# fabianschenk/REVO

Measured on AMD Instinct MI355X. Metric: tracked frames/sec at 640x480, 4-level pyramid; ATE vs reference, higher is better.
Workload: dtype f32

## Files before the change

### profiles/stream_busy.py

```python
import collections
import sqlite3
import statistics
import sys

db = sqlite3.connect(sys.argv[1])
cols = [r[1] for r in db.execute("pragma table_info(kernels)")]
sid = "stream_id" if "stream_id" in cols else "queue_id"
rows = list(db.execute("select name, start, end, %s from kernels order by start" % sid))
short = lambda n: n.replace("(anonymous namespace)::", "").replace("void ", "").split("(")[0]
trk = [i for i, r in enumerate(rows) if "k_track<false>" in r[0]]
first = int(sys.argv[2]) if len(sys.argv) > 2 else 14
count = int(sys.argv[3]) if len(sys.argv) > 3 else 30
t_idx = trk[first:first + count]
t0, t1 = rows[t_idx[0]][1], rows[t_idx[-1]][1]
nsteps = len(t_idx) - 1
print("%d steps between tracker launches %d and %d: %.1f us per step" % (nsteps, first, first + count - 1, (t1 - t0) / 1e3 / nsteps))
busy = collections.defaultdict(float)
dur = collections.defaultdict(list)
by = collections.defaultdict(list)
for n, s, e, q in rows:
    if t0 <= s < t1:
        busy[q] += (e - s) / 1e3
        dur[short(n)].append((e - s) / 1e3)
        by[q].append((s, e, short(n)))
for q in sorted(busy):
    names = collections.Counter(x[2] for x in by[q]).most_common(2)
    print("stream %-3s busy %6.1f us per step  (%s)" % (q, busy[q] / nsteps, ", ".join(n for n, _ in names)))
print("kernel                         per step   avg us   min     max")
for k, v in sorted(dur.items(), key=lambda kv: -sum(kv[1])):
    print("%-30s %6.2f   %7.1f %7.1f %7.1f" % (k, len(v) / nsteps, statistics.mean(v), min(v), max(v)))
print("idle gap in front of a kernel on its own stream (mean / max us):")
for q in sorted(by):
    gaps = collections.defaultdict(list)
    for a, b in zip(by[q], by[q][1:]):
        gaps[b[2]].append((b[0] - a[1]) / 1e3)
    print("  stream %-3s %s" % (q, {k: (round(statistics.mean(v), 1), round(max(v), 1)) for k, v in gaps.items()}))
```

### revo_amd/csrc/revo_dev.h

```cpp
#pragma once
#include <hip/hip_runtime.h>
#include <stdint.h>
#include "../../include/revo_hip.h"

#define REVO_L REVO_MAX_LEVELS

struct LevelGeom {
  int w, h;
  int npix;
  float fx, fy, cx, cy;
  int patch;
  int hist_w, hist_h;
  int nchunk;
  int chunk_rows;
  int wpr;
  int nms_block_base;
  int has_orig;
  int pix_base;
  int edt_rows;
  int edt_block_base;
  int strip_base;
  int cc_base;
  int band_rows, nbands, band_base;
};

struct PyrGeom {
  int frame0;
  int fstride;
  int n_levels;
  int total_nms_blocks, total_pix, total_edt_blocks, total_strips, total_cc;
  int total_bands, any_banded;
  int hyst_force;
  int hyst_heavy_runs;
  int total_tiles;
  int pts_staged;
  float depth_min, depth_max;
  int canny_low, canny_high;
  int use_edge_hist;
  float n_percentage;
  double fill_thr[REVO_L];
  LevelGeom lv[REVO_L];
};

struct FramePlanes {
  uint8_t* gray[REVO_L];
  float* depth[REVO_L];
  uint2* cs[REVO_L];
  uint8_t* edges[REVO_L];
  uint8_t* edges_orig[REVO_L];
  int* scratch[REVO_L];
  float4* pts[REVO_L];
  float4* pts_trk[REVO_L];
  float* dt[REVO_L];
  float4* table[REVO_L];
  uint8_t* hist[REVO_L];
  int* chunk[REVO_L];
  unsigned* cmask[REVO_L];
  uint8_t* vb[REVO_L];
  int* npts;
  int* hist_nz;
  int* strip_tot;
  uint32_t* ebits[REVO_L];
  int* need_full;
  int* hyst_heavy;
  int* tile_base;
  float* stage[REVO_L];
  unsigned short* epre[REVO_L];
  int* stage_base;
};

struct PairDesc {
  const float4* pts[REVO_L];
  const int* npts;
  const float* dt[REVO_L];
  float R[9];
  float T[3];
};

struct TrackParams {
  int pyr_min_lvl, pyr_max_lvl;
  int lvl_begin, lvl_end;
  int check_init;
  int eval_only;
  int kspec[REVO_L];
  int redundant_n;
  float lambda_success_fac, lambda_fail_fac;
  float lambda_initial[REVO_L], step_size_min[REVO_L], convergence_eps[REVO_L];
  int max_its[REVO_L];
  float edge_distance[REVO_L];
  float huber_edge;
  int use_edge_filter;
  struct { float fx, fy, cx, cy; int w, h; } cam[REVO_L];
  int exact_sums;
};

struct EvalOut {
  float A[36];
  float b[6];
  float error;
  float mean_err;
  float sum_w, sum_u;
  int good, bad;
};

#define REVO_MAX_WIDTH 2048
#define NMS_ROWS 6
#define EDT_ROW_PX 1280
#ifndef REVO_HYST_LDS_MAX
#define REVO_HYST_LDS_MAX 158720
#endif
#ifndef TRACK_THREADS
#define TRACK_THREADS 512
#endif
#ifndef TRACK_MAX_CLUSTER
#define TRACK_MAX_CLUSTER 32
#endif
#define TRACK_KMAX 4
#define TRACK_NVAL 48
#define TRACK_NVAL_X 132
#define TRACK_MAIL_NVAL TRACK_NVAL_X

void launch_gray_depth(const PyrGeom& g, const FramePlanes& p, const uint8_t* d_bgr, const float* d_depth_f32,
                       const uint16_t* d_depth_u16, float u16_alpha, int B, hipStream_t s);
void launch_pyrdown(const PyrGeom& g, const FramePlanes& p, int lvl, int B, hipStream_t s, int parts = 3, bool stage_edges = false);
void launch_edge_prefix(const PyrGeom& g, const FramePlanes& p, int B, hipStream_t s);
void launch_canny_nms(const PyrGeom& g, const FramePlanes& p, int B, hipStream_t s);
void launch_hyst(const PyrGeom& g, const FramePlanes& p, int B, hipStream_t s);
void launch_fill(const PyrGeom& g, const FramePlanes& p, int B, hipStream_t s);
void launch_compact(const PyrGeom& g, const FramePlanes& p, int B, hipStream_t s);
void launch_tile_points(const PyrGeom& g, const FramePlanes& p, int B, hipStream_t s, int which = 3);
void launch_pyrdown_bgr(const uint8_t* src, int w, int h, uint8_t* dst, hipStream_t s);
void launch_colored_pcl(const PyrGeom& g, const FramePlanes& p, int frame, int lvl, int dense, const uint8_t* bgr_lvl,
                        int* chunk, unsigned* cmask, int* total, int cap, float* out8, hipStream_t s);
void launch_keyframe(const PyrGeom& g, const FramePlanes& p, int f0, int fstride, int count, hipStream_t s, int which = 3);
int launch_track(const PairDesc* d_descs, const TrackParams& prm, revo_pair_result* d_out, EvalOut* d_eval,
                 int n_pairs, unsigned long long* d_mail, unsigned* epoch_io, int cluster, unsigned* d_resident, hipStream_t s);
void launch_track_gate(unsigned* d_resident, unsigned want, hipStream_t s);
int launch_track_one(const PairDesc& desc, const TrackParams& prm, revo_pair_result* out, EvalOut* eval_out,
                     unsigned long long* d_mail, unsigned* epoch_io, int cluster, unsigned* seq_ptr, unsigned seq_val,
                     unsigned* d_resident, hipStream_t s);
void launch_solve6(const float* d_Ab , int n, float* d_x , hipStream_t s);
int track_blocks_per_cu();
void launch_grad_table(const PyrGeom& g, const FramePlanes& p, int f0, int fstride, int count, hipStream_t s);
struct VoteArgs { float RT[3][12]; const float4* pts[3]; const int* n[3]; };
void launch_vote(const PyrGeom& g, const FramePlanes& curr, int curr_frame, int lvl, int n_clouds, const VoteArgs& va,
                 int* d_marks , int* d_hist8 , unsigned* d_done ,
                 int* h_out8 , unsigned seq_val, int use_orig_edges,
                 hipStream_t s);
void launch_copy_cloud(float4* dst, const float4* src, int* dst_n, const int* src_n, hipStream_t s);
struct VoteDesc {
  float RT[3][12]; const float4* pts[3]; const int* n[3]; int n_clouds;
  const uint8_t* edges; const float* depth;
  int* marks; int* hist8; unsigned* done;
  int* host_out;
};
struct CloudCopyDesc { float4* dst; const float4* src; int* dst_n; const int* src_n; };
struct CopySeg { const void* src; void* dst; size_t bytes; };
void launch_vote_multi(const PyrGeom& g, int lvl, int n, const VoteDesc* d_descs, unsigned seq_val, hipStream_t s);
void launch_copy_cloud_multi(int n, const CloudCopyDesc* d_descs, hipStream_t s);
void launch_copy_segments(int n, const CopySeg* d_segs, hipStream_t s);

#define INFO_THREADS 256
#define INFO_CHUNK 1024
#define INFO_MAX_GROUPS 32
#define INFO_PART_DOUBLES 64
struct InfoParams {
  float fx, fy, cx, cy;
  int w, h;
  float edge_distance, huber_edge;
  int use_edge_filter, level;
};
static inline int info_groups(int npix) {
  const int g = (npix + 8 * INFO_CHUNK - 1) / (8 * INFO_CHUNK);
  return g < 1 ? 1 : (g > INFO_MAX_GROUPS ? INFO_MAX_GROUPS : g);
}
void launch_pair_info(const PairDesc* d_descs, const void* d_pose, int pose_stride, int flag_word, const InfoParams& prm,
                      int n_pairs, double* d_part, int* d_cnt, unsigned* d_ticket, revo_pair_info* d_out, hipStream_t s);
```

### revo_amd/csrc/revo_pyramid.hip

```cpp
#include "revo_dev.h"
#include <type_traits>

namespace {

#ifdef REVO_BUILD_PRIO
#define BUILD_PRIO() __builtin_amdgcn_s_setprio(REVO_BUILD_PRIO)
#else
#define BUILD_PRIO()
#endif

__device__ __forceinline__ int level_of(const PyrGeom& g, int v, int LevelGeom::*base) {
  int l = 0;
#pragma unroll
  for (int k = 1; k < REVO_L; ++k)
    if (k < g.n_levels && v >= g.lv[k].*base) l = k;
  return l;
}
__device__ __forceinline__ int clampi(int v, int lo, int hi) { return v < lo ? lo : (v > hi ? hi : v); }
__device__ __forceinline__ int reflect101(int i, int n) {
  if (i < 0) i = -i;
  if (i >= n) i = 2 * n - 2 - i;
  return i;
}

// ... 199 lines not shown
    lo[k] = __builtin_amdgcn_perm(as_u32(dy), as_u32(dx), 0x05040100u);
    hi[k] = __builtin_amdgcn_perm(as_u32(dy), as_u32(dx), 0x07060302u);
  }
  const uint32_t rv = valid ? ~0u : 0u;
#define MAG2(x) __builtin_amdgcn_sdot2(as_s2(x), as_s2(x), 0, false)
  m.v0 = MAG2(lo[0]) & (int)(cm_left & rv);
  m.v1 = MAG2(hi[0]) & (int)rv;
  m.v2 = MAG2(lo[1]) & (int)rv;
  m.v3 = MAG2(hi[1]) & (int)rv;
  m.v4 = MAG2(lo[2]) & (int)rv;
  m.v5 = MAG2(hi[2]) & (int)(cm_right & rv);
#undef MAG2
  dxy.v0 = hi[0]; dxy.v1 = lo[1]; dxy.v2 = hi[1]; dxy.v3 = lo[2];
}
__device__ __forceinline__ void nms_row4(const MRow4& A, const MRow4& B, const MRow4& C, const DRow4& d, int low, int high,
                                         uint32_t* cand, uint32_t* strong) {
  uint32_t cb = 0, sb = 0;
  nms_px(0, A.v0, A.v1, A.v2, B.v0, B.v1, B.v2, C.v0, C.v1, C.v2, d.v0, low, high, cb, sb);
  nms_px(1, A.v1, A.v2, A.v3, B.v1, B.v2, B.v3, C.v1, C.v2, C.v3, d.v1, low, high, cb, sb);
  nms_px(2, A.v2, A.v3, A.v4, B.v2, B.v3, B.v4, C.v2, C.v3, C.v4, d.v2, low, high, cb, sb);
  nms_px(3, A.v3, A.v4, A.v5, B.v3, B.v4, B.v5, C.v3, C.v4, C.v5, d.v3, low, high, cb, sb);
  *cand = cb;
  *strong = sb;
}
__global__ void __launch_bounds__(256) k_canny_nms4(PyrGeom g, FramePlanes pl) {
  BUILD_PRIO();
  const int f = g.frame0 + blockIdx.z;
  if (blockIdx.x == 0 && threadIdx.x < REVO_L) {
    pl.need_full[f * REVO_L + threadIdx.x] = 0;
    pl.hist_nz[f * REVO_L + threadIdx.x] = 0;
  }
  const int l = level_of(g, blockIdx.x, &LevelGeom::nms_block_base);
  const LevelGeom& lv = g.lv[l];
  const int w = lv.w, h = lv.h;
  const int rt = 8 * lv.wpr;
  const int t = (blockIdx.x - lv.nms_block_base) * 256 + threadIdx.x;
  const int yb = t / rt, xg = t - yb * rt;
  const int y0 = yb * NMS_R;
  if (y0 >= h) return;
  const int x = xg * 4;
  const bool active = x < w;
  const uint8_t* gray = pl.gray[l] + (size_t)f * lv.npix;
  const bool has_prev = x > 0, has_next = x + 4 < w;
  const int xo = active ? x : 0;
  const int o_prev = (active && has_prev) ? xo - 4 : xo, o_next = (active && has_next) ? xo + 4 : xo;
  const uint32_t cm_left = (active && has_prev) ? ~0u : 0u, cm_right = (active && has_next) ? ~0u : 0u;
  struct Raw { uint32_t prev, m0, next; };
  auto load_raw = [&](int r) -> Raw {
    const int rr = clampi(r, 0, h - 1);
    const uint8_t* row = gray + (size_t)rr * w;
    Raw q;
    q.m0 = *reinterpret_cast<const uint32_t*>(row + xo);
    q.prev = *reinterpret_cast<const uint32_t*>(row + o_prev);
    q.next = *reinterpret_cast<const uint32_t*>(row + o_next);
    return q;
  };
  auto make_hrow = [&](Raw q) -> HRow4 {
    if (!has_prev) q.prev = (q.m0 & 0xffu) * 0x01010101u;
    if (!has_next) q.next = (q.m0 >> 24) * 0x01010101u;
    return hrow4(q.prev, q.m0, q.next);
  };
  HRow4 H0, H1, H2;
  MRow4 M0, M1, M2;
  DRow4 D0, D1, D2;
  {
    const Raw r0 = load_raw(y0 - 2), r1 = load_raw(y0 - 1), r2 = load_raw(y0), r3 = load_raw(y0 + 1);
    H0 = make_hrow(r0); H1 = make_hrow(r1); H2 = make_hrow(r2);
    mag_row4(H0, H1, H2, cm_left, cm_right, active && y0 - 1 >= 0, M0, D0);
    H0 = make_hrow(r3);
  }
  Raw ahead = load_raw(y0 + 2);
  mag_row4(H1, H2, H0, cm_left, cm_right, active, M1, D1);
  uint2* out = pl.cs[l] + ((size_t)f * h + y0) * lv.wpr + (xg >> 3);
  const int sh = 4 * (threadIdx.x & 7);
  auto emit = [&](int i, uint32_t cb, uint32_t sb) {
    uint32_t cw = cb << sh, sw = sb << sh;
    cw |= (uint32_t)__builtin_amdgcn_update_dpp(0, (int)cw, 0xB1, 0xf, 0xf, true);
    sw |= (uint32_t)__builtin_amdgcn_update_dpp(0, (int)sw, 0xB1, 0xf, 0xf, true);
    cw |= (uint32_t)__builtin_amdgcn_update_dpp(0, (int)cw, 0x4E, 0xf, 0xf, true);
    sw |= (uint32_t)__builtin_amdgcn_update_dpp(0, (int)sw, 0x4E, 0xf, 0xf, true);
    cw |= (uint32_t)__builtin_amdgcn_update_dpp(0, (int)cw, 0x141, 0xf, 0xf, true);
    sw |= (uint32_t)__builtin_amdgcn_update_dpp(0, (int)sw, 0x141, 0xf, 0xf, true);
    if ((threadIdx.x & 7) == 0 && y0 + i < h) out[(size_t)i * lv.wpr] = make_uint2(cw, sw);
  };
#define NMS_STEP4(i, Ha, Hb, Hc, Ma, Mb, Mc, Db, Dc)                                  \
  {                                                                                   \
    Hc = make_hrow(ahead);                                                            \
    if ((i) < NMS_R - 1) ahead = load_raw(y0 + (i) + 3);                              \
    mag_row4(Ha, Hb, Hc, cm_left, cm_right, active && y0 + (i) + 1 < h, Mc, Dc);      \
    uint32_t cb, sb;                                                                  \
    nms_row4(Ma, Mb, Mc, Db, g.canny_low, g.canny_high, &cb, &sb);                    \
    emit((i), cb, sb);                                                                \
  }
  NMS_STEP4(0, H2, H0, H1, M0, M1, M2, D1, D2)
  NMS_STEP4(1, H0, H1, H2, M1, M2, M0, D2, D0)
  NMS_STEP4(2, H1, H2, H0, M2, M0, M1, D0, D1)
  NMS_STEP4(3, H2, H0, H1, M0, M1, M2, D1, D2)
  NMS_STEP4(4, H0, H1, H2, M1, M2, M0, D2, D0)
  NMS_STEP4(5, H1, H2, H0, M2, M0, M1, D0, D1)
#undef NMS_STEP4
}

#ifndef HYST_THREADS
#define HYST_THREADS 1024
#endif
__device__ __forceinline__ uint32_t dil3(uint32_t a, uint32_t al, uint32_t ar) {
  return a | __builtin_amdgcn_alignbit(a, al, 31) | __builtin_amdgcn_alignbit(ar, a, 1);
}
__device__ __forceinline__ uint32_t run_fill(uint32_t C, uint32_t S) {
  const uint32_t up = ((C + S) ^ C) & C;
  const uint32_t rC = __builtin_bitreverse32(C), rS = __builtin_bitreverse32(S);
  const uint32_t dn = __builtin_bitreverse32(((rC + rS) ^ rC) & rC);
  return up | dn | S;
}

#ifdef REVO_HYST_PROFILE
#define HP(i) if (threadIdx.x == 0) hp[i] = clock64()
#define HA(i) if (threadIdx.x == 0) { const long long now_ = clock64(); ha[i] += now_ - hlast; hlast = now_; }
#else
#define HP(i)
#define HA(i)
#endif
template <bool C_IN_LDS, bool E_GLOBAL = false>
__device__ __forceinline__ void hyst_level(const PyrGeom& g, const FramePlanes& pl, const int l, const int f, uint32_t* s_mem) {
  static_assert(!(C_IN_LDS && E_GLOBAL), "the candidate bitmap is in LDS only when the edge bitmap is");
#ifdef REVO_HYST_PROFILE
  long long hp[12], ha[8], hlast = 0;
  for (int i = 0; i < 12; ++i) hp[i] = 0;
  for (int i = 0; i < 8; ++i) ha[i] = 0;
  int dbg_sweeps = 0, dbg_bands = 0;
#endif
  HP(0);
  const LevelGeom& lv = g.lv[l];
  const int w = lv.w, h = lv.h, wpr = lv.wpr;
  const int pitch = wpr;
  const int nwords = h * wpr;
  const int e_words = (h + 2) * pitch + 2;
  uint32_t* Cl = s_mem;
  uint32_t* Ebase = C_IN_LDS ? s_mem + (REVO_HYST_LDS_MAX / 4 - e_words)
                  : (E_GLOBAL ? reinterpret_cast<uint32_t*>(pl.scratch[l] + (size_t)f * g.lv[l].npix) : s_mem);
  uint32_t* E = Ebase + 1;
  const uint2* cs = pl.cs[l] + (size_t)f * h * wpr;
  const int tid = threadIdx.x;
  for (int i = tid; i < pitch + 1; i += HYST_THREADS) { Ebase[i] = 0u; Ebase[e_words - 1 - i] = 0u; }
  for (int i = tid; i < nwords; i += HYST_THREADS) {
    const uint2 v = cs[i];
    E[pitch + i] = v.y;
    if (C_IN_LDS) Cl[i] = v.x & ~v.y;
  }
  __syncthreads();
  HP(1);
  bool done = false;
#ifdef REVO_HYST_PROFILE
  int dbg_runs = -1, dbg_t = 0, dbg_a = 0;
#endif
  if (C_IN_LDS) {
    unsigned short* Bs = reinterpret_cast<unsigned short*>(Cl + nwords);
    uint32_t* parent = Cl + nwords + (nwords + 2) / 2;
    const int table_words = (int)(REVO_HYST_LDS_MAX / 4) - (nwords + (nwords + 2) / 2);
    const int cap = min(table_words / 2, table_words - e_words);
    const int cap_keep = (table_words - e_words) / 2;
    __shared__ int s_wsum[HYST_THREADS / 64];
    __shared__ int s_total, s_promoted;
#ifdef REVO_HYST_PROFILE
    __shared__ int s_dbg[4];
    if (tid < 4) s_dbg[tid] = 0;
#endif
    auto weak = [&](int wi) -> uint32_t { return Cl[wi]; };
    auto starts = [](uint32_t wk) -> uint32_t { return wk & ~(wk << 1); };
    const float inv_wpr = 1.0f / (float)wpr;
    const uint32_t FLAG = 0x80000000u, IDM = 0x7fffffffu;
#ifdef REVO_HYST_PROFILE
    hlast = clock64();
#endif
    for (int sweep = 0; sweep < 64 && !done; ++sweep) {
#ifdef REVO_HYST_PROFILE
      ++dbg_sweeps;
#endif
      {
        const int wpt = (nwords + HYST_THREADS - 1) / HYST_THREADS;
        const int w0 = min(nwords, tid * wpt), w1 = min(nwords, w0 + wpt);
        int mine = 0;
        for (int wi = w0; wi < w1; ++wi) mine += __popc(starts(weak(wi)));
        int incl = mine;
#pragma unroll
        for (int o = 1; o < 64; o <<= 1) {
          const int v = __shfl_up(incl, o);
          if ((tid & 63) >= o) incl += v;
        }
        __syncthreads();
        if ((tid & 63) == 63) s_wsum[tid >> 6] = incl;
        if (tid == 0) s_promoted = 0;
        __syncthreads();
        int before = incl - mine;
        for (int k = 0; k < (tid >> 6); ++k) before += s_wsum[k];
        if (tid == HYST_THREADS - 1) { s_total = before + mine; Bs[nwords] = (unsigned short)min(65535, before + mine); }
        for (int wi = w0; wi < w1; ++wi) {
          Bs[wi] = (unsigned short)before;
          before += __popc(starts(weak(wi)));
        }
        __syncthreads();
      }
      const int nruns = s_total;
      HA(0);
#ifdef REVO_HYST_PROFILE
      if (sweep == 0) dbg_runs = nruns;
#endif
      if (nruns >= 65536 || cap < 64) break;
      if (nruns == 0) { done = true; break; }
      int nb = (nruns + cap - 1) / cap, band_rows = h;
      for (;; ++nb) {
        band_rows = (h + nb - 1) / nb;
        bool fits = true;
        for (int r0 = 0; r0 < h; r0 += band_rows)
          fits = fits && ((int)Bs[min(h, r0 + band_rows) * wpr] - (int)Bs[r0 * wpr] <= cap);
        if (fits || band_rows == 1) break;
      }
      if (band_rows == 1 && nb > h) break;
      for (int r0 = 0; r0 < h; r0 += band_rows) {
        const int wa = r0 * wpr, wb = min(h, r0 + band_rows) * wpr;
        const int id0 = Bs[wa], nr = (int)Bs[wb] - id0;
        if (nr == 0) continue;
        uint32_t* rec = parent + nr;
        auto id_of = [&](int wi, int bit) -> int { return (int)Bs[wi] - id0 + __popc(starts(weak(wi)) & ((2u << bit) - 1u)) - 1; };
        auto key_of = [](int x) -> uint32_t { return ((((uint32_t)x * 40503u) >> 1) & 0x7fffu) << 16 | (uint32_t)x; };
        auto find = [&](int x) -> int {
          uint32_t p2 = parent[x] & IDM;
          while ((int)(p2 & 0xffffu) != x) {
            const uint32_t gp = parent[p2 & 0xffffu] & IDM;
            if (gp != p2) atomicMin(&parent[x], gp);
            x = (int)(p2 & 0xffffu); p2 = gp;
          }
          return x;
        };
        auto unite = [&](int a2, int b2) {
          for (;;) {
            a2 = find(a2); b2 = find(b2);
            if (a2 == b2) return;
            uint32_t ka = key_of(a2), kb = key_of(b2);
            if (ka > kb) { const int t2 = a2; a2 = b2; b2 = t2; const uint32_t t3 = ka; ka = kb; kb = t3; }
            const uint32_t old = atomicMin(&parent[b2], ka);
            if (old == kb) return;
            b2 = (int)(old & 0xffffu);
          }
        };
        auto run_at = [&](int i, int* wi_out, uint32_t* run_out) {
          const uint32_t rc = rec[i];
          *wi_out = (int)(rc >> 10);
          *run_out = (0xffffffffu >> (31u - (rc & 31u))) << ((rc >> 5) & 31u);
        };
        for (int wi = wa + tid; wi < wb; wi += HYST_THREADS) {
          int me = (int)Bs[wi] - id0;
          const uint32_t wk = weak(wi);
          for (uint32_t m = starts(wk); m; m &= m - 1, ++me) {
            const int bit = __ffs(m) - 1;
            const uint32_t t2 = ~(wk >> bit);
            const int len = t2 ? __ffs(t2) - 1 : 32 - bit;
            parent[me] = key_of(me);
            rec[me] = ((uint32_t)wi << 10) | ((uint32_t)bit << 5) | (uint32_t)(len - 1);
          }
        }
        __syncthreads();
        HA(1);
#ifdef REVO_HYST_PROFILE
        ++dbg_bands;
#endif
        for (int me = tid; me < nr; me += HYST_THREADS) {
          int wi; uint32_t run;
          run_at(me, &wi, &run);
          int r = (int)(((float)wi + 0.5f) * inv_wpr);
          r += (r + 1) * wpr <= wi ? 1 : (r * wpr > wi ? -1 : 0);
          const int c = wi - r * wpr;
          if ((run & 1u) && c > 0 && (weak(wi - 1) >> 31)) unite(me, id_of(wi - 1, 31));
          if (r == r0) continue;
          for (uint32_t a2 = weak(wi - wpr) & (run | (run << 1) | (run >> 1)); a2;) {
            const int ab = __ffs(a2) - 1;
            a2 &= ~(a2 & ~(a2 + (1u << ab)));
            unite(me, id_of(wi - wpr, ab));
          }
          if ((run & 1u) && c > 0 && (weak(wi - wpr - 1) >> 31)) unite(me, id_of(wi - wpr - 1, 31));
          if ((run >> 31) && c < wpr - 1 && (weak(wi - wpr + 1) & 1u)) unite(me, id_of(wi - wpr + 1, 0));
        }
        __syncthreads();
        HA(2);
        for (int me = tid; me < nr; me += HYST_THREADS) parent[me] = key_of(find(me));
        __syncthreads();
        HA(3);
        if (nr > cap_keep) {
          for (int i = tid; i < pitch + 1; i += HYST_THREADS) { Ebase[i] = 0u; Ebase[e_words - 1 - i] = 0u; }
          for (int i0 = tid; i0 < nwords; i0 += 5 * HYST_THREADS) {
            uint2 v[5];
#pragma unroll
            for (int k = 0; k < 5; ++k) v[k] = cs[min(i0 + k * HYST_THREADS, nwords - 1)];
#pragma unroll
            for (int k = 0; k < 5; ++k) {
              const int i = i0 + k * HYST_THREADS;
              if (i < nwords) E[pitch + i] = v[k].y | (v[k].x & ~Cl[i]);
            }
          }
          __syncthreads();
        }
        HA(6);
        for (int wi = wa + tid; wi < wb; wi += HYST_THREADS) {
          const uint32_t wk = weak(wi);
          if (!wk) continue;
          int r = (int)(((float)wi + 0.5f) * inv_wpr);
          r += (r + 1) * wpr <= wi ? 1 : (r * wpr > wi ? -1 : 0);
          const int c = wi - r * wpr;
          const uint32_t lm = c > 0 ? ~0u : 0u, rm = c < wpr - 1 ? ~0u : 0u;
          const uint32_t* Xc = E + pitch + wi;
          const uint32_t sd = dil3(Xc[-pitch], Xc[-pitch - 1] & lm, Xc[-pitch + 1] & rm) | dil3(Xc[pitch], Xc[pitch - 1] & lm, Xc[pitch + 1] & rm) |
                              __builtin_amdgcn_alignbit(Xc[0], Xc[-1] & lm, 31) | __builtin_amdgcn_alignbit(Xc[1] & rm, Xc[0], 1);
          if (!(wk & sd)) continue;
          const uint32_t touched = run_fill(wk, wk & sd);
          int me = (int)Bs[wi] - id0;
          for (uint32_t m = starts(wk); m; m &= m - 1, ++me)
            if (touched & m & (0u - m)) {
              uint32_t* root = &parent[parent[me] & 0xffffu];
#ifdef REVO_HYST_PROFILE
              atomicAdd(&s_dbg[0], 1);
              if (!(*root & FLAG)) atomicAdd(&s_dbg[1], 1);
#endif
              if (!(*root & FLAG)) atomicOr(root, FLAG);
            }
        }
        __syncthreads();
        HA(4);
#ifdef REVO_HYST_PROFILE
        dbg_t = s_dbg[0]; dbg_a = s_dbg[1];
#endif
        bool any = false;
        for (int wi = wa + tid; wi < wb; wi += HYST_THREADS) {
          const uint32_t wk = weak(wi);
          if (!wk) continue;
          int me = (int)Bs[wi] - id0;
          uint32_t prom = 0;
          for (uint32_t m = starts(wk); m; m &= m - 1, ++me)
            if (parent[parent[me] & 0xffffu] & FLAG) prom |= m & (0u - m);
          if (!prom) continue;
          const uint32_t runs = run_fill(wk, prom);
          Cl[wi] = wk & ~runs;
          E[pitch + wi] |= runs;
          any = any || (r0 > 0 && wi < wa + wpr);
        }
        if (any) s_promoted = 1;
        __syncthreads();
        HA(5);
      }
      if (nb == 1 || !s_promoted) done = true;
    }
    __syncthreads();
  }
  if (!done) {
    __shared__ unsigned short s_list[HYST_THREADS];
    __shared__ unsigned char s_act[2][HYST_THREADS];
    __shared__ int s_n;
  const int max_strips = HYST_THREADS / wpr;
  const int rpt = (h + max_strips - 1) / max_strips;
  const int nstrips = (h + rpt - 1) / rpt;
  const int n_items = nstrips * wpr;
  s_act[0][tid] = 0; s_act[1][tid] = 0;
  if (tid == 0) s_n = 0;
  __syncthreads();
  int n_list = n_items;
#ifndef REVO_HYST_MAXIT
#define REVO_HYST_MAXIT 8192
#endif
  for (int it = 0; it < REVO_HYST_MAXIT; ++it) {
    const int wb = it & 1;
    bool changed = false;
    if (tid < n_list) {
      const int item = it == 0 ? tid : (int)s_list[tid];
      const int strip = item / wpr, c = item - strip * wpr;
      const int r0 = strip * rpt, r1 = min(h, r0 + rpt) - 1;
      uint32_t* Ec = E + pitch + c;
      const uint32_t lm = c > 0 ? ~0u : 0u, rm = c < wpr - 1 ? ~0u : 0u;
      auto Cat = [&](int r) -> uint32_t { return C_IN_LDS ? (Cl[r * wpr + c] | Ec[r * pitch]) : cs[r * wpr + c].x; };
      uint32_t prev_d = dil3(Ec[(r0 - 1) * pitch], Ec[(r0 - 1) * pitch - 1] & lm, Ec[(r0 - 1) * pitch + 1] & rm);
      uint32_t cur = Ec[r0 * pitch], cl = Ec[r0 * pitch - 1] & lm, cr = Ec[r0 * pitch + 1] & rm;
      for (int r = r0; r <= r1; ++r) {
        const uint32_t nx = Ec[(r + 1) * pitch], nl = Ec[(r + 1) * pitch - 1] & lm, nr = Ec[(r + 1) * pitch + 1] & rm;
        const uint32_t Cw = Cat(r);
        const uint32_t hz = __builtin_amdgcn_alignbit(cur, cl, 31) | __builtin_amdgcn_alignbit(cr, cur, 1);
        const uint32_t F = run_fill(Cw, cur | (Cw & (prev_d | dil3(nx, nl, nr) | hz)));
        if (F != cur) { Ec[r * pitch] = F; changed = true; }
        prev_d = dil3(F, cl, cr);
        cur = nx; cl = nl; cr = nr;
      }
      prev_d = dil3(cur, cl, cr);
      cur = Ec[r1 * pitch]; cl = Ec[r1 * pitch - 1] & lm; cr = Ec[r1 * pitch + 1] & rm;
      for (int r = r1; r >= r0; --r) {
        const uint32_t nx = Ec[(r - 1) * pitch], nl = Ec[(r - 1) * pitch - 1] & lm, nr = Ec[(r - 1) * pitch + 1] & rm;
        const uint32_t Cw = Cat(r);
        const uint32_t hz = __builtin_amdgcn_alignbit(cur, cl, 31) | __builtin_amdgcn_alignbit(cr, cur, 1);
        const uint32_t F = run_fill(Cw, cur | (Cw & (prev_d | dil3(nx, nl, nr) | hz)));
        if (F != cur) { Ec[r * pitch] = F; changed = true; }
        prev_d = dil3(F, cl, cr);
        cur = nx; cl = nl; cr = nr;
      }
      if (changed) s_act[wb][item] = 1;
    }
    if (!__syncthreads_or(changed ? 1 : 0)) break;
    bool act = false;
    if (tid < n_items) {
      const int strip = tid / wpr, c = tid - strip * wpr;
      const unsigned char* a = s_act[wb];
#pragma unroll
      for (int ds = -1; ds <= 1; ++ds)
#pragma unroll
        for (int dc = -1; dc <= 1; ++dc) {
          const int ss = strip + ds, cc = c + dc;
          if (ss >= 0 && ss < nstrips && cc >= 0 && cc < wpr) act = act || a[ss * wpr + cc] != 0;
        }
    }
    const unsigned long long m = __ballot(act);
    int base = 0;
    if ((tid & 63) == 0 && m) base = atomicAdd(&s_n, __popcll(m));
    base = __shfl(base, 0);
    if (act) s_list[base + __popcll(m & ((1ull << (tid & 63)) - 1ull))] = (unsigned short)tid;
    s_act[wb ^ 1][tid] = 0;
    __syncthreads();
    n_list = s_n;
    __syncthreads();
    if (tid == 0) s_n = 0;
  }
  __syncthreads();
  }
  __syncthreads();
  HP(5);
  uint8_t* edges = pl.edges[l] + (size_t)f * lv.npix;
  uint8_t* orig = lv.has_orig ? pl.edges_orig[l] + (size_t)f * lv.npix : nullptr;
  const bool rows16 = (w & 15) == 0;
  const float inv_w = 1.0f / (float)w;
  for (int i = tid; i < lv.npix / 16; i += HYST_THREADS) {
    const int p = i * 16;
    int y = (int)(((float)p + 0.5f) * inv_w);
    y += (y + 1) * w <= p ? 1 : (y * w > p ? -1 : 0);
    const int x = p - y * w;
    uint32_t o[4];
    if (rows16) {
      const uint32_t bits = (E[(y + 1) * pitch + (x >> 5)] >> (x & 31)) & 0xffffu;
#pragma unroll
      for (int q = 0; q < 4; ++q) o[q] = ((((bits >> (4 * q)) & 0xfu) * 0x00204081u) & 0x01010101u) * 0xffu;
    } else {
#pragma unroll
      for (int q = 0; q < 4; ++q) {
        int xx = x + 4 * q, yy = y;
        while (xx >= w) { xx -= w; yy += 1; }
        const uint32_t bits = (E[(yy + 1) * pitch + (xx >> 5)] >> (xx & 31)) & 0xfu;
        o[q] = ((bits * 0x00204081u) & 0x01010101u) * 0xffu;
      }
    }
    const uint4 v = make_uint4(o[0], o[1], o[2], o[3]);
    *reinterpret_cast<uint4*>(edges + p) = v;
    if (orig) *reinterpret_cast<uint4*>(orig + p) = v;
  }
  {
    uint2* csw = pl.cs[l] + (size_t)f * h * wpr;
    for (int i = tid; i < nwords; i += HYST_THREADS) csw[i].y = E[pitch + i];
  }
  HP(6);
  if (lv.patch > 0) {
    const int ntiles = lv.hist_w * lv.hist_h;
    int nz = 0;
    const float inv_hw = 1.0f / (float)lv.hist_w;
    for (int t0 = 0; t0 < ntiles; t0 += HYST_THREADS) {
      const int t = t0 + tid;
      if (t < ntiles) {
        int ty = (int)(((float)t + 0.5f) * inv_hw);
        ty += (ty + 1) * lv.hist_w <= t ? 1 : (ty * lv.hist_w > t ? -1 : 0);
        const int tx = t - ty * lv.hist_w;
        const int xa = tx * lv.patch, xb = xa + lv.patch;
        const int wa = xa >> 5, wb = (xb - 1) >> 5;
        const uint32_t ma = ~0u << (xa & 31), mb = (xb & 31) ? ~0u >> (32 - (xb & 31)) : ~0u;
        const uint32_t m0 = wa == wb ? ma & mb : ma, m1 = wb > wa + 1 ? ~0u : (wb > wa ? mb : 0u), m2 = wb > wa + 1 ? mb : 0u;
        const int o1 = wb > wa ? 1 : 0, o2 = wb > wa + 1 ? 2 : 0;
        const uint32_t* row = E + (ty * lv.patch + 1) * pitch + wa;
        int cnt = 0;
        for (int y = 0; y < lv.patch; ++y, row += pitch) cnt += __popc(row[0] & m0) + __popc(row[o1] & m1) + __popc(row[o2] & m2);
        const uint8_t v = (uint8_t)(cnt & 255);
        pl.hist[l][(size_t)f * ntiles + t] = v;
        nz += v != 0;
      }
    }
    __shared__ int s_nz;
    if (tid == 0) s_nz = 0;
    __syncthreads();
    if (nz) atomicAdd(&s_nz, nz);
    __syncthreads();
    if (tid == 0) pl.hist_nz[f * REVO_L + l] = s_nz;
  }
#ifdef REVO_HYST_PROFILE
  HP(7);
  if (threadIdx.x == 0 && l == 0 && f < 64)
    printf("hyst f=%d: load %lld uf_total %lld [scan %lld record %lld link %lld compress %lld flag %lld resolve %lld] runs %d sweeps %d bands %d uf %d rebuild %lld out %lld hist %lld touched %d atomics %d\n", f,
           hp[1] - hp[0], hp[5] - hp[1], ha[0], ha[1], ha[2], ha[3], ha[4], ha[5], dbg_runs, dbg_sweeps, dbg_bands, (int)done, ha[6], hp[6] - hp[5], hp[7] - hp[6], dbg_t, dbg_a);
#endif
}
template <bool C_IN_LDS, bool E_GLOBAL = false>
__global__ void __launch_bounds__(HYST_THREADS) k_hyst(PyrGeom g, FramePlanes pl, int only_flagged, int n_frames) {
  BUILD_PRIO();
  extern __shared__ uint32_t s_mem[];
  const int n_items = g.n_levels * n_frames;
  if (only_flagged) {
    __shared__ int s_any;
    if (threadIdx.x == 0) s_any = 0;
    __syncthreads();
    for (int item = threadIdx.x; item < n_items; item += HYST_THREADS)
      if (pl.need_full[(g.frame0 + item % n_frames) * REVO_L + item / n_frames]) s_any = 1;
    __syncthreads();
    if (!s_any) return;
  }
  for (int item = blockIdx.x; item < n_items; item += gridDim.x) {
    const int l = item / n_frames;
    const int f = g.frame0 + item % n_frames;
    if (only_flagged && !pl.need_full[f * REVO_L + l]) continue;
    hyst_level<C_IN_LDS, E_GLOBAL>(g, pl, l, f, s_mem);
    __syncthreads();
  }
}

#ifndef HB_THREADS
#define HB_THREADS 1024
#endif
#ifndef HB_LDS_WORDS
#define HB_LDS_WORDS 16384
#endif
struct BandRef { int l, R0, R1; };
__device__ __forceinline__ BandRef band_ref(const PyrGeom& g, int bi) {
  int l = 0;
#pragma unroll
  for (int k = 1; k < REVO_L; ++k)
    if (k < g.n_levels && bi >= g.lv[k].band_base) l = k;
  const LevelGeom& lv = g.lv[l];
  const int b = bi - lv.band_base;
  BandRef r;
  r.l = l; r.R0 = b * lv.band_rows; r.R1 = min(lv.h, r.R0 + lv.band_rows);
  return r;
}
__device__ __forceinline__ int band_capb(const LevelGeom& lv) {
  const int hb = lv.band_rows, nwb = hb * lv.wpr;
  const int table_words = HB_LDS_WORDS - (nwb + (nwb + 2) / 2);
  const int e_words = (hb + 2) * lv.wpr + 2;
  int cap = min(table_words / 2, table_words - e_words);
  cap = min(cap, 65535);
  const int h_last = lv.h - (lv.nbands - 1) * lv.band_rows;
  cap = min(cap, ((h_last * lv.w - 4 - 2 * lv.wpr) / 8) * 5);
  return max(cap, 0) & ~31;
}
struct BandRec { int* hdr; int* bs_first; int* bs_last; uint32_t* flags; unsigned short* root; uint32_t* rec; };
__device__ __forceinline__ BandRec band_rec(const FramePlanes& pl, const LevelGeom& lv, int l, int f, int R0, int capb) {
  int* base = pl.scratch[l] + (size_t)f * lv.npix + (size_t)R0 * lv.w;
  BandRec r;
  r.hdr = base; r.bs_first = base + 4; r.bs_last = base + 4 + lv.wpr;
  r.flags = reinterpret_cast<uint32_t*>(base + 4 + 2 * lv.wpr);
  r.root = reinterpret_cast<unsigned short*>(base + 4 + 2 * lv.wpr + capb / 32);
  r.rec = reinterpret_cast<uint32_t*>(base + 4 + 2 * lv.wpr + capb / 32 + capb / 2);
  return r;
}

__device__ __forceinline__ void hyst_band(const PyrGeom& g, const FramePlanes& pl, const BandRef br, const int f, uint32_t* s_mem) {
  __shared__ int s_wsum[HB_THREADS / 64];
  __shared__ int s_total;
  const int l = br.l;
  const LevelGeom& lv = g.lv[l];
  const int h = lv.h, wpr = lv.wpr, pitch = wpr;
  const int hb = br.R1 - br.R0, nwb = hb * wpr, e_words = (hb + 2) * pitch + 2;
  const int tid = threadIdx.x;
  uint32_t* Cl = s_mem;
  uint32_t* Ebase = s_mem + (HB_LDS_WORDS - e_words);
  uint32_t* E = Ebase + 1;
  const uint2* cs = pl.cs[l] + ((size_t)f * h + br.R0) * wpr;
  const int capb = band_capb(lv);
  const BandRec rec_out = band_rec(pl, lv, l, f, br.R0, capb);
  auto load_e = [&](bool with_cl) {
    if (tid == 0) { Ebase[0] = 0u; Ebase[e_words - 1] = 0u; }
    for (int c = tid; c < wpr; c += HB_THREADS) {
      E[c] = br.R0 > 0 ? cs[c - wpr].y : 0u;
      E[(hb + 1) * pitch + c] = br.R1 < h ? cs[nwb + c].y : 0u;
    }
    for (int i0 = tid; i0 < nwb; i0 += 4 * HB_THREADS) {
      uint2 v[4];
#pragma unroll
      for (int k = 0; k < 4; ++k) v[k] = cs[min(i0 + k * HB_THREADS, nwb - 1)];
#pragma unroll
      for (int k = 0; k < 4; ++k) {
        const int i = i0 + k * HB_THREADS;
        if (i < nwb) {
          if (with_cl) { E[pitch + i] = v[k].y; Cl[i] = v[k].x & ~v[k].y; }
          else E[pitch + i] = v[k].y | (v[k].x & ~Cl[i]);
        }
      }
    }
  };
  load_e(true);
  __syncthreads();
  unsigned short* Bs = reinterpret_cast<unsigned short*>(Cl + nwb);
  uint32_t* parent = Cl + nwb + (nwb + 2) / 2;
  const int table_words = HB_LDS_WORDS - (nwb + (nwb + 2) / 2);
  const int cap_keep = (table_words - e_words) / 2;
  auto starts = [](uint32_t wk) -> uint32_t { return wk & ~(wk << 1); };
  const float inv_wpr = 1.0f / (float)wpr;
  const uint32_t FLAG = 0x80000000u, IDM = 0x7fffffffu;
  {
    const int wpt = (nwb + HB_THREADS - 1) / HB_THREADS;
    const int w0 = min(nwb, tid * wpt), w1 = min(nwb, w0 + wpt);
    int mine = 0;
    for (int wi = w0; wi < w1; ++wi) mine += __popc(starts(Cl[wi]));
    int incl = mine;
#pragma unroll
    for (int o = 1; o < 64; o <<= 1) {
      const int v = __shfl_up(incl, o);
      if ((tid & 63) >= o) incl += v;
    }
    if ((tid & 63) == 63) s_wsum[tid >> 6] = incl;
    __syncthreads();
    int before = incl - mine;
    for (int k = 0; k < (tid >> 6); ++k) before += s_wsum[k];
    if (tid == HB_THREADS - 1) { s_total = before + mine; Bs[nwb] = (unsigned short)min(65535, before + mine); }
    for (int wi = w0; wi < w1; ++wi) {
      Bs[wi] = (unsigned short)before;
      before += __popc(starts(Cl[wi]));
    }
    __syncthreads();
  }
  const int nr = s_total;
  if (nr > capb) {
    if (tid == 0) { pl.need_full[f * REVO_L + l] = 1; rec_out.hdr[0] = 0; rec_out.hdr[1] = 0; rec_out.hdr[2] = 0; }
    return;
  }
  uint32_t* rec = parent + nr;
  if (nr > 0) {
    auto id_of = [&](int wi, int bit) -> int { return (int)Bs[wi] + __popc(starts(Cl[wi]) & ((2u << bit) - 1u)) - 1; };
    auto key_of = [](int x) -> uint32_t { return ((((uint32_t)x * 40503u) >> 1) & 0x7fffu) << 16 | (uint32_t)x; };
    auto find = [&](int x) -> int {
      uint32_t p2 = parent[x] & IDM;
      while ((int)(p2 & 0xffffu) != x) {
        const uint32_t gp = parent[p2 & 0xffffu] & IDM;
        if (gp != p2) atomicMin(&parent[x], gp);
        x = (int)(p2 & 0xffffu); p2 = gp;
      }
      return x;
    };
    auto unite = [&](int a2, int b2) {
      for (;;) {
        a2 = find(a2); b2 = find(b2);
        if (a2 == b2) return;
        uint32_t ka = key_of(a2), kb = key_of(b2);
        if (ka > kb) { const int t2 = a2; a2 = b2; b2 = t2; const uint32_t t3 = ka; ka = kb; kb = t3; }
// ... 1298 lines not shown
```

Baseline: 114,500.

## Replace atomic union-find linking in hysteresis with forest build plus pointer jumping

For large bands, the hysteresis connected-component step no longer unites every run with all of its neighbours through atomic union-find. Each run first points at a single neighbour, which builds a forest, and the forest is flattened by synchronous pointer-jumping rounds. Only junction runs, those with more than one neighbour, are collected into an LDS list and united afterwards, followed by another round of jumps. The goal is fewer atomics and less serial find chasing. In exchange the change adds block-wide synchronisation per jump round, and falls back to the iterative path when the jumping does not converge.

```diff
diff --git a/profiles/hyst_link_premise.py b/profiles/hyst_link_premise.py
--- /dev/null
+++ b/profiles/hyst_link_premise.py
@@ -0,0 +1,37 @@
+import os
+import pathlib
+import sys
+import tempfile
+
+import numpy as np
+
+ROOT = os.path.dirname(os.path.dirname(os.path.abspath(__file__)))
+sys.path[:0] = [ROOT, os.path.join(ROOT, "tests")]
+import hyst_link_cases as hc
+from oracle import ro
+from revo_amd import synth
+from revo_amd.settings import ImgPyramidSettings
+
+
+def main():
+    tmp = pathlib.Path(tempfile.mkdtemp())
+    exe = hc.build_host(tmp)
+    s = ImgPyramidSettings.scaled(640, 480, 4, hist_patch=(20, 10, 5, 0, 0, 0))
+    cases, names = [], []
+    for seed in range(int(sys.argv[1]) if len(sys.argv) > 1 else 32):
+        p = synth.make_pair(seed, s)
+        for k in ("ref", "curr"):
+            gray = ro.bgr2gray(p[k][0])
+            cand, strong = hc.nms(gray)
+            if seed < 2:
+                assert np.array_equal(hc.flood(cand, strong), ro.canny(gray) > 0), "the suppression differs from the oracle's"
+            cases.append((hc.words(cand & ~strong), hc.words(strong), 0, 64, 2048))
+            names.append("%d %s" % (seed, k))
+    print("frame      runs junctions share depth votes(forest, roots) serial  link == flood fill")
+    for name, (got, want, st) in zip(names, hc.run_host(exe, tmp, cases)):
+        print("%-8s %6d %9d %5.3f %5d %6d %6d %6d  %s" % (name, st["runs"], st["junctions"], st["junctions"] / max(1, st["runs"]), st["depth"],
+                                                      st["rounds1"], st["rounds2"], st["serial"], np.array_equal(got, want)))
+
+
+if __name__ == "__main__":
+    main()
diff --git a/profiles/stream_busy.py b/profiles/stream_busy.py
--- a/profiles/stream_busy.py
+++ b/profiles/stream_busy.py
@@ -8,7 +8,7 @@
 sid = "stream_id" if "stream_id" in cols else "queue_id"
 rows = list(db.execute("select name, start, end, %s from kernels order by start" % sid))
 short = lambda n: n.replace("(anonymous namespace)::", "").replace("void ", "").split("(")[0]
-trk = [i for i, r in enumerate(rows) if "k_track<false>" in r[0]]
+trk = [i for i, r in enumerate(rows) if "k_track<" in r[0]]
 first = int(sys.argv[2]) if len(sys.argv) > 2 else 14
 count = int(sys.argv[3]) if len(sys.argv) > 3 else 30
 t_idx = trk[first:first + count]
diff --git a/revo_amd/csrc/revo_dev.h b/revo_amd/csrc/revo_dev.h
--- a/revo_amd/csrc/revo_dev.h
+++ b/revo_amd/csrc/revo_dev.h
@@ -1,7 +1,107 @@
 #pragma once
+#include <stdint.h>
+#ifndef REVO_HYST_LINK_HOST
 #include <hip/hip_runtime.h>
-#include <stdint.h>
 #include "../../include/revo_hip.h"
+#endif
+
+#ifdef REVO_HYST_LINK_HOST
+#define HYST_FN static inline
+static inline int hyst_popc(uint32_t v) { return __builtin_popcount(v); }
+static inline int hyst_ffs(uint32_t v) { return __builtin_ffs((int)v); }
+static inline uint32_t hyst_atomic_min(uint32_t* p, uint32_t v) { const uint32_t o = *p; if (v < o) *p = v; return o; }
+#else
+#define HYST_FN __device__ __forceinline__
+__device__ __forceinline__ int hyst_popc(uint32_t v) { return __popc(v); }
+__device__ __forceinline__ int hyst_ffs(uint32_t v) { return __ffs(v); }
+__device__ __forceinline__ uint32_t hyst_atomic_min(uint32_t* p, uint32_t v) { return atomicMin(p, v); }
+#endif
+#define HYST_JUNCTION 0x80000000u
+#define HYST_JUMP_ROUNDS 20
+#define HYST_JUMPS_PER_VOTE 8
+#define HYST_SERIAL_RUNS 3
+
+HYST_FN uint32_t hyst_starts(uint32_t wk) { return wk & ~(wk << 1); }
+HYST_FN uint32_t hyst_key(int x) { return ((((uint32_t)x * 40503u) >> 1) & 0x7fffu) << 16 | (uint32_t)x; }
+HYST_FN int hyst_row(int wi, int wpr, float inv_wpr) {
+  int r = (int)(((float)wi + 0.5f) * inv_wpr);
+  r += (r + 1) * wpr <= wi ? 1 : (r * wpr > wi ? -1 : 0);
+  return r;
+}
+HYST_FN void hyst_run_at(uint32_t rc, int* wi, uint32_t* run) {
+  *wi = (int)((rc & ~HYST_JUNCTION) >> 10);
+  *run = (0xffffffffu >> (31u - (rc & 31u))) << ((rc >> 5) & 31u);
+}
+struct HystWords { uint32_t wl, wu, wul, wur; int bl, bu, bul, bur; };
+HYST_FN HystWords hyst_words(const uint32_t* Cl, const unsigned short* Bs, int wi, int wpr, float inv_wpr, int r0, int id0) {
+  const int r = hyst_row(wi, wpr, inv_wpr), c = wi - r * wpr;
+  const bool up = r > r0, left = c > 0, right = c < wpr - 1;
+  const int il = left ? wi - 1 : wi, iu = up ? wi - wpr : wi, iul = up && left ? wi - wpr - 1 : wi, iur = up && right ? wi - wpr + 1 : wi;
+  HystWords q;
+  q.wl = Cl[il]; q.wu = Cl[iu]; q.wul = Cl[iul]; q.wur = Cl[iur];
+  q.bl = (int)Bs[il] - id0; q.bu = (int)Bs[iu] - id0; q.bul = (int)Bs[iul] - id0; q.bur = (int)Bs[iur] - id0;
+  if (!left) q.wl = 0u;
+  if (!up) q.wu = 0u;
+  if (!(up && left)) q.wul = 0u;
+  if (!(up && right)) q.wur = 0u;
+  return q;
+}
+struct HystNb { uint32_t above; int p, d, r; };
+HYST_FN HystNb hyst_neighbours(uint32_t run, const HystWords& q) {
+  HystNb n;
+  n.p = (run & 1u) && (q.wl >> 31) ? q.bl + hyst_popc(hyst_starts(q.wl)) - 1 : -1;
+  uint32_t a = q.wu & (run | (run << 1) | (run >> 1));
+  if (n.p >= 0 && (a & 1u)) a &= a + 1u;
+  n.above = a;
+  n.d = (run & 1u) && n.p < 0 && !(q.wu & 1u) && (q.wul >> 31) ? q.bul + hyst_popc(hyst_starts(q.wul)) - 1 : -1;
+  n.r = (run >> 31) && !(q.wu >> 31) && (q.wur & 1u) ? q.bur : -1;
+  return n;
+}
+HYST_FN int hyst_id_above(const HystWords& q, int bit) { return q.bu + hyst_popc(hyst_starts(q.wu) & ((2u << bit) - 1u)) - 1; }
+HYST_FN uint32_t hyst_first_parent(int me, uint32_t run, const HystWords& q, bool* junction) {
+  const HystNb n = hyst_neighbours(run, q);
+  const int count = (n.p >= 0) + hyst_popc(hyst_starts(n.above)) + (n.d >= 0) + (n.r >= 0);
+  *junction = count > 1;
+  const int first = n.p >= 0 ? n.p : (n.above ? hyst_id_above(q, hyst_ffs(n.above) - 1) : (n.d >= 0 ? n.d : (n.r >= 0 ? n.r : me)));
+  return hyst_key(first);
+}
+HYST_FN bool hyst_jump(uint32_t* parent, int me, uint32_t p, uint32_t gp) {
+  if (gp == p) return false;
+  parent[me] = gp;
+  return true;
+}
+HYST_FN int hyst_find(uint32_t* parent, int x) {
+  uint32_t p2 = parent[x];
+  while ((int)(p2 & 0xffffu) != x) {
+    const uint32_t gp = parent[p2 & 0xffffu];
+    if (gp != p2) hyst_atomic_min(&parent[x], gp);
+    x = (int)(p2 & 0xffffu); p2 = gp;
+  }
+  return x;
+}
+HYST_FN void hyst_unite(uint32_t* parent, int a2, int b2) {
+  for (;;) {
+    a2 = hyst_find(parent, a2); b2 = hyst_find(parent, b2);
+    if (a2 == b2) return;
+    uint32_t ka = hyst_key(a2), kb = hyst_key(b2);
+    if (ka > kb) { const int t2 = a2; a2 = b2; b2 = t2; const uint32_t t3 = ka; ka = kb; kb = t3; }
+    const uint32_t old = hyst_atomic_min(&parent[b2], ka);
+    if (old == kb) return;
+    b2 = (int)(old & 0xffffu);
+  }
+}
+HYST_FN void hyst_unite_all(uint32_t* parent, int me, uint32_t run, const HystWords& q) {
+  const HystNb n = hyst_neighbours(run, q);
+  if (n.p >= 0) hyst_unite(parent, me, n.p);
+  for (uint32_t a2 = n.above; a2;) {
+    const int ab = hyst_ffs(a2) - 1;
+    a2 &= ~(a2 & ~(a2 + (1u << ab)));
+    hyst_unite(parent, me, hyst_id_above(q, ab));
+  }
+  if (n.d >= 0) hyst_unite(parent, me, n.d);
+  if (n.r >= 0) hyst_unite(parent, me, n.r);
+}
+#ifndef REVO_HYST_LINK_HOST
 
 #define REVO_L REVO_MAX_LEVELS
 
@@ -176,3 +276,4 @@
 }
 void launch_pair_info(const PairDesc* d_descs, const void* d_pose, int pose_stride, int flag_word, const InfoParams& prm,
                       int n_pairs, double* d_part, int* d_cnt, unsigned* d_ticket, revo_pair_info* d_out, hipStream_t s);
+#endif
diff --git a/revo_amd/csrc/revo_pyramid.hip b/revo_amd/csrc/revo_pyramid.hip
--- a/revo_amd/csrc/revo_pyramid.hip
+++ b/revo_amd/csrc/revo_pyramid.hip
@@ -375,8 +375,10 @@
   HP(1);
   bool done = false;
 #ifdef REVO_HYST_PROFILE
-  int dbg_runs = -1, dbg_t = 0, dbg_a = 0;
+  int dbg_runs = -1, dbg_t = 0, dbg_a = 0, dbg_nj = 0;
 #endif
+  __shared__ unsigned short s_list[2 * HYST_THREADS];
+  unsigned char (*s_act)[HYST_THREADS] = reinterpret_cast<unsigned char (*)[HYST_THREADS]>(s_list + HYST_THREADS);
   if (C_IN_LDS) {
     unsigned short* Bs = reinterpret_cast<unsigned short*>(Cl + nwords);
     uint32_t* parent = Cl + nwords + (nwords + 2) / 2;
@@ -384,7 +386,8 @@
     const int cap = min(table_words / 2, table_words - e_words);
     const int cap_keep = (table_words - e_words) / 2;
     __shared__ int s_wsum[HYST_THREADS / 64];
-    __shared__ int s_total, s_promoted;
+    __shared__ int s_total, s_promoted, s_nj;
+    bool bailed = false;
 #ifdef REVO_HYST_PROFILE
     __shared__ int s_dbg[4];
     if (tid < 4) s_dbg[tid] = 0;
@@ -392,7 +395,7 @@
     auto weak = [&](int wi) -> uint32_t { return Cl[wi]; };
     auto starts = [](uint32_t wk) -> uint32_t { return wk & ~(wk << 1); };
     const float inv_wpr = 1.0f / (float)wpr;
-    const uint32_t FLAG = 0x80000000u, IDM = 0x7fffffffu;
+    const uint32_t FLAG = 0x80000000u;
 #ifdef REVO_HYST_PROFILE
     hlast = clock64();
 #endif
@@ -445,33 +448,7 @@
         const int id0 = Bs[wa], nr = (int)Bs[wb] - id0;
         if (nr == 0) continue;
         uint32_t* rec = parent + nr;
-        auto id_of = [&](int wi, int bit) -> int { return (int)Bs[wi] - id0 + __popc(starts(weak(wi)) & ((2u << bit) - 1u)) - 1; };
-        auto key_of = [](int x) -> uint32_t { return ((((uint32_t)x * 40503u) >> 1) & 0x7fffu) << 16 | (uint32_t)x; };
-        auto find = [&](int x) -> int {
-          uint32_t p2 = parent[x] & IDM;
-          while ((int)(p2 & 0xffffu) != x) {
-            const uint32_t gp = parent[p2 & 0xffffu] & IDM;
-            if (gp != p2) atomicMin(&parent[x], gp);
-            x = (int)(p2 & 0xffffu); p2 = gp;
-          }
-          return x;
-        };
-        auto unite = [&](int a2, int b2) {
-          for (;;) {
-            a2 = find(a2); b2 = find(b2);
-            if (a2 == b2) return;
-            uint32_t ka = key_of(a2), kb = key_of(b2);
-            if (ka > kb) { const int t2 = a2; a2 = b2; b2 = t2; const uint32_t t3 = ka; ka = kb; kb = t3; }
-            const uint32_t old = atomicMin(&parent[b2], ka);
-            if (old == kb) return;
-            b2 = (int)(old & 0xffffu);
-          }
-        };
-        auto run_at = [&](int i, int* wi_out, uint32_t* run_out) {
-          const uint32_t rc = rec[i];
-          *wi_out = (int)(rc >> 10);
-          *run_out = (0xffffffffu >> (31u - (rc & 31u))) << ((rc >> 5) & 31u);
-        };
+        if (tid == 0) s_nj = 0;
         for (int wi = wa + tid; wi < wb; wi += HYST_THREADS) {
           int me = (int)Bs[wi] - id0;
           const uint32_t wk = weak(wi);
@@ -479,7 +456,7 @@
             const int bit = __ffs(m) - 1;
             const uint32_t t2 = ~(wk >> bit);
             const int len = t2 ? __ffs(t2) - 1 : 32 - bit;
-            parent[me] = key_of(me);
+            parent[me] = hyst_key(me);
             rec[me] = ((uint32_t)wi << 10) | ((uint32_t)bit << 5) | (uint32_t)(len - 1);
           }
         }
@@ -488,27 +465,99 @@
 #ifdef REVO_HYST_PROFILE
         ++dbg_bands;
 #endif
-        for (int me = tid; me < nr; me += HYST_THREADS) {
-          int wi; uint32_t run;
-          run_at(me, &wi, &run);
-          int r = (int)(((float)wi + 0.5f) * inv_wpr);
-          r += (r + 1) * wpr <= wi ? 1 : (r * wpr > wi ? -1 : 0);
-          const int c = wi - r * wpr;
-          if ((run & 1u) && c > 0 && (weak(wi - 1) >> 31)) unite(me, id_of(wi - 1, 31));
-          if (r == r0) continue;
-          for (uint32_t a2 = weak(wi - wpr) & (run | (run << 1) | (run >> 1)); a2;) {
-            const int ab = __ffs(a2) - 1;
-            a2 &= ~(a2 & ~(a2 + (1u << ab)));
-            unite(me, id_of(wi - wpr, ab));
+        if (nr <= HYST_SERIAL_RUNS * HYST_THREADS) {
+          for (int me = tid; me < nr; me += HYST_THREADS) {
+            int wi; uint32_t run;
+            hyst_run_at(rec[me], &wi, &run);
+            hyst_unite_all(parent, me, run, hyst_words(Cl, Bs, wi, wpr, inv_wpr, r0, id0));
           }
-          if ((run & 1u) && c > 0 && (weak(wi - wpr - 1) >> 31)) unite(me, id_of(wi - wpr - 1, 31));
-          if ((run >> 31) && c < wpr - 1 && (weak(wi - wpr + 1) & 1u)) unite(me, id_of(wi - wpr + 1, 0));
+          __syncthreads();
+          HA(2);
+          for (int me = tid; me < nr; me += HYST_THREADS) parent[me] = hyst_key(hyst_find(parent, me));
+          __syncthreads();
+          HA(3);
+        } else {
+        constexpr int HL_UNROLL = 2, HJ_UNROLL = 4;
+        constexpr int HL_LIST = 2 * HYST_THREADS;
+        for (int base = tid; base < nr + tid; base += HL_UNROLL * HYST_THREADS) {
+          uint32_t rc[HL_UNROLL], run[HL_UNROLL];
+          HystWords q[HL_UNROLL];
+#pragma unroll
+          for (int k = 0; k < HL_UNROLL; ++k) rc[k] = rec[min(base + k * HYST_THREADS, nr - 1)];
+#pragma unroll
+          for (int k = 0; k < HL_UNROLL; ++k) {
+            int wi;
+            hyst_run_at(rc[k], &wi, &run[k]);
+            q[k] = hyst_words(Cl, Bs, wi, wpr, inv_wpr, r0, id0);
+          }
+#pragma unroll
+          for (int k = 0; k < HL_UNROLL; ++k) {
+            const int me = base + k * HYST_THREADS;
+            bool junction = false;
+            const uint32_t key = hyst_first_parent(me, run[k], q[k], &junction);
+            junction = junction && me < nr;
+            if (me < nr) parent[me] = key;
+            const unsigned long long jm = __ballot(junction);
+            if (jm) {
+              int slot = 0;
+              if ((tid & 63) == 0) slot = atomicAdd(&s_nj, __popcll(jm));
+              slot = __shfl(slot, 0) + __popcll(jm & ((1ull << (tid & 63)) - 1ull));
+              if (junction) {
+                if (slot < HL_LIST) s_list[slot] = (unsigned short)me;
+                else rec[me] = rc[k] | HYST_JUNCTION;
+              }
+            }
+          }
         }
         __syncthreads();
         HA(2);
-        for (int me = tid; me < nr; me += HYST_THREADS) parent[me] = key_of(find(me));
-        __syncthreads();
+        auto jump_all = [&]() -> bool {
+          for (int round = 0; round < HYST_JUMP_ROUNDS; ++round) {
+            bool changed = true;
+            for (int pass = 0; pass < HYST_JUMPS_PER_VOTE && changed; ++pass) {
+              changed = false;
+              for (int base = tid; base < nr; base += HJ_UNROLL * HYST_THREADS) {
+                uint32_t p[HJ_UNROLL], gp[HJ_UNROLL];
+#pragma unroll
+                for (int k = 0; k < HJ_UNROLL; ++k) p[k] = parent[min(base + k * HYST_THREADS, nr - 1)];
+#pragma unroll
+                for (int k = 0; k < HJ_UNROLL; ++k) gp[k] = parent[p[k] & 0xffffu];
+#pragma unroll
+                for (int k = 0; k < HJ_UNROLL; ++k)
+                  if (base + k * HYST_THREADS < nr) changed = hyst_jump(parent, base + k * HYST_THREADS, p[k], gp[k]) || changed;
+              }
+            }
+            if (!__syncthreads_or(changed ? 1 : 0)) return true;
+          }
+          return false;
+        };
+        bool flat = jump_all();
         HA(3);
+        const int nj = s_nj;
+#ifdef REVO_HYST_PROFILE
+        dbg_nj = max(dbg_nj, nj);
+#endif
+        if (flat && nj > 0) {
+          for (int j = tid; j < min(nj, HL_LIST); j += HYST_THREADS) {
+            const int me = (int)s_list[j];
+            int wi; uint32_t run;
+            hyst_run_at(rec[me], &wi, &run);
+            hyst_unite_all(parent, me, run, hyst_words(Cl, Bs, wi, wpr, inv_wpr, r0, id0));
+          }
+          if (nj > HL_LIST)
+            for (int me = tid; me < nr; me += HYST_THREADS) {
+              const uint32_t rc = rec[me];
+              if (!(rc & HYST_JUNCTION)) continue;
+              int wi; uint32_t run;
+              hyst_run_at(rc, &wi, &run);
+              hyst_unite_all(parent, me, run, hyst_words(Cl, Bs, wi, wpr, inv_wpr, r0, id0));
+            }
+          __syncthreads();
+          flat = jump_all();
+        }
+        bailed = !flat;
+        HA(7);
+        }
         if (nr > cap_keep) {
           for (int i = tid; i < pitch + 1; i += HYST_THREADS) { Ebase[i] = 0u; Ebase[e_words - 1 - i] = 0u; }
           for (int i0 = tid; i0 < nwords; i0 += 5 * HYST_THREADS) {
@@ -524,6 +573,7 @@
           __syncthreads();
         }
         HA(6);
+        if (bailed) break;
         for (int wi = wa + tid; wi < wb; wi += HYST_THREADS) {
           const uint32_t wk = weak(wi);
           if (!wk) continue;
@@ -570,13 +620,12 @@
         __syncthreads();
         HA(5);
       }
+      if (bailed) break;
       if (nb == 1 || !s_promoted) done = true;
     }
     __syncthreads();
   }
   if (!done) {
-    __shared__ unsigned short s_list[HYST_THREADS];
-    __shared__ unsigned char s_act[2][HYST_THREADS];
     __shared__ int s_n;
   const int max_strips = HYST_THREADS / wpr;
   const int rpt = (h + max_strips - 1) / max_strips;
@@ -716,8 +765,8 @@
 #ifdef REVO_HYST_PROFILE
   HP(7);
   if (threadIdx.x == 0 && l == 0 && f < 64)
-    printf("hyst f=%d: load %lld uf_total %lld [scan %lld record %lld link %lld compress %lld flag %lld resolve %lld] runs %d sweeps %d bands %d uf %d rebuild %lld out %lld hist %lld touched %d atomics %d\n", f,
-           hp[1] - hp[0], hp[5] - hp[1], ha[0], ha[1], ha[2], ha[3], ha[4], ha[5], dbg_runs, dbg_sweeps, dbg_bands, (int)done, ha[6], hp[6] - hp[5], hp[7] - hp[6], dbg_t, dbg_a);
+    printf("hyst f=%d: load %lld uf_total %lld [scan %lld record %lld forest %lld jump %lld junctions %lld flag %lld resolve %lld] runs %d junctions %d sweeps %d bands %d uf %d rebuild %lld out %lld hist %lld touched %d atomics %d\n", f,
+           hp[1] - hp[0], hp[5] - hp[1], ha[0], ha[1], ha[2], ha[3], ha[7], ha[4], ha[5], dbg_runs, dbg_nj, dbg_sweeps, dbg_bands, (int)done, ha[6], hp[6] - hp[5], hp[7] - hp[6], dbg_t, dbg_a);
 #endif
 }
 template <bool C_IN_LDS, bool E_GLOBAL = false>
```

After: 114,400. Within noise of the previous version (-0.0%).
